# bgmanuel99/Super-Resolution-Images-for-3D-Printing-Defect-Detection

Hardware: AMD Instinct MI355X
Metric: 4x-SR MPix/s on 512x512 LR batch (higher is better)
Workload: dtype bf16

## Files before the change

super-resolution-images-for-3d-printing-defect-detection_amd/csrc/attention.hip:

```cpp
#include "common.h"

#include <cstdlib>

namespace {

constexpr int KV_TILE = 64;

template <typename T> struct AT;
template <> struct AT<float>  { static constexpr int PITCH = KV_TILE * 4 + 4; };

struct AttnParams {
    const char* qkv; int64_t cs; int qoff, koff, voff;
    char* o; int64_t o_cs; int o_coff;
    int N;
    const float* knorm;
};

__device__ __forceinline__ float xhalf(float v) { return __shfl_xor(v, 32); }

__global__ void __launch_bounds__(256, 2) attn_f32_kernel(AttnParams p) {
    constexpr int PITCH = AT<float>::PITCH;
    __shared__ __attribute__((aligned(16))) char vt[32 * PITCH];

    const int tid = threadIdx.x, lane = tid & 63, wave = tid >> 6, r = lane & 31, h = lane >> 5;
    const int b = blockIdx.y;
    const int N = p.N;
    const float* base = reinterpret_cast<const float*>(p.qkv) + (int64_t)b * N * p.cs;
    const int q = blockIdx.x * 128 + wave * 32 + r;
    const int qc = q < N ? q : N - 1;

    float qf[4];
    {
        const float* qp = base + (int64_t)qc * p.cs + p.qoff;
#pragma unroll
        for (int j = 0; j < 4; ++j) qf[j] = qp[2 * j + h];
    }

    f32x16 oacc;
#pragma unroll
    for (int e = 0; e < 16; ++e) oacc[e] = 0.f;
    float m_run = -INFINITY, l_run = 0.f;

    const int skey = tid >> 2, soct = tid & 3;

    for (int k0 = 0; k0 < N; k0 += KV_TILE) {
        __syncthreads();
        {
            const int key = k0 + skey;
            const float* vp = base + (int64_t)(key < N ? key : N - 1) * p.cs + p.voff + soct * 8;
            f32x4 v0 = *reinterpret_cast<const f32x4*>(vp), v1 = *reinterpret_cast<const f32x4*>(vp + 4);
#pragma unroll
            for (int e = 0; e < 4; ++e) {
                *reinterpret_cast<float*>(vt + (soct * 8 + e) * PITCH + skey * 4) = v0[e];
                *reinterpret_cast<float*>(vt + (soct * 8 + 4 + e) * PITCH + skey * 4) = v1[e];
            }
        }
        __syncthreads();
#pragma unroll
        for (int sub = 0; sub < KV_TILE / 32; ++sub) {
            const int kb = k0 + sub * 32;
            if (kb >= N) break;
            f32x16 s;
#pragma unroll
            for (int e = 0; e < 16; ++e) s[e] = 0.f;
            {
                const int key = kb + r;
                const float* kp = base + (int64_t)(key < N ? key : N - 1) * p.cs + p.koff;
#pragma unroll
                for (int j = 0; j < 4; ++j) s = __builtin_amdgcn_mfma_f32_32x32x2f32(kp[2 * j + h], qf[j], s, 0, 0, 0);
            }
            float mx = -INFINITY;
#pragma unroll
            for (int i = 0; i < 16; ++i) {
                const int key = kb + (i & 3) + 8 * (i >> 2) + 4 * h;
                if (key >= N) s[i] = -INFINITY;
                mx = fmaxf(mx, s[i]);
            }
            mx = fmaxf(mx, xhalf(mx));
            const float m_new = fmaxf(m_run, mx);
            const float alpha = __expf(m_run - m_new);
            float psum = 0.f;
#pragma unroll
            for (int i = 0; i < 16; ++i) { s[i] = __expf(s[i] - m_new); psum += s[i]; }
            l_run = l_run * alpha + psum;
            m_run = m_new;
#pragma unroll
            for (int e = 0; e < 16; ++e) oacc[e] *= alpha;
#pragma unroll
            for (int i = 0; i < 16; ++i) {
                const int krow = sub * 32 + (i & 3) + 8 * (i >> 2);
                const float va = *reinterpret_cast<const float*>(vt + r * PITCH + (krow + 4 * h) * 4);
                oacc = __builtin_amdgcn_mfma_f32_32x32x2f32(va, s[i], oacc, 0, 0, 0);
            }
        }
    }
    const float l_tot = l_run + xhalf(l_run);
    const float inv = 1.f / l_tot;
    if (q < N) {
        float* op = reinterpret_cast<float*>(p.o) + ((int64_t)b * N + q) * p.o_cs + p.o_coff;
#pragma unroll
        for (int g = 0; g < 4; ++g) {
            const int d0 = 8 * g + 4 * h;
            f32x4 t = {oacc[4 * g] * inv, oacc[4 * g + 1] * inv, oacc[4 * g + 2] * inv, oacc[4 * g + 3] * inv};
            *reinterpret_cast<f32x4*>(op + d0) = t;
        }
    }
}

constexpr int KT2 = 128;
constexpr int PITCH2 = KT2 * 2 + 8;

__global__ void __launch_bounds__(64) attn_knorm_kernel(const bf16_t* qkv, int64_t cs, int koff, int N, int ngroups, float* out) {
    const int g = blockIdx.x % ngroups, b = blockIdx.x / ngroups, lane = threadIdx.x;
    const bf16_t* base = qkv + (int64_t)b * N * cs + koff;
    float m = 0.f;
#pragma unroll
    for (int t = 0; t < 2; ++t) {
        const int key = g * 128 + t * 64 + lane;
        if (key < N) {
            const bf16x8 k = *reinterpret_cast<const bf16x8*>(base + (int64_t)key * cs);
            float n2 = 0.f;
#pragma unroll
            for (int e = 0; e < 8; ++e) n2 += (float)k[e] * (float)k[e];
            m = fmaxf(m, n2);
        }
    }
#pragma unroll
    for (int o = 32; o > 0; o >>= 1) m = fmaxf(m, __shfl_xor(m, o));
    if (lane == 0) out[(int64_t)b * ngroups + g] = sqrtf(m);
}

template <int QB>
__global__ void __launch_bounds__(256, 3) attn_bf16_kernel(AttnParams p) {
    __shared__ __attribute__((aligned(16))) char vt[32 * PITCH2];
    const int tid = threadIdx.x, lane = tid & 63, wave = tid >> 6, r = lane & 31, h = lane >> 5;
    const int N = p.N;
    constexpr int QW = 64 * QB * 2;
    const int nqt = (N + QW - 1) / QW;
    const int b = blockIdx.x / nqt, qt = blockIdx.x - b * nqt;
    const bf16_t* base = reinterpret_cast<const bf16_t*>(p.qkv) + (int64_t)b * N * p.cs;
    const int cs = (int)p.cs;
    int qi[QB];
    bf16x8 qb[QB];
#pragma unroll
    for (int j = 0; j < QB; ++j) {
        qi[j] = qt * QW + wave * (32 * QB) + j * 32 + r;
        const int qc = qi[j] < N ? qi[j] : N - 1;
        bf16x8 z = {};
        qb[j] = z;
        if (h == 0) qb[j] = *reinterpret_cast<const bf16x8*>(base + (int64_t)qc * cs + p.qoff);
    }
    float qn2 = 0.f;
#pragma unroll
    for (int j = 0; j < QB; ++j) {
        float n2 = 0.f;
#pragma unroll
        for (int e = 0; e < 8; ++e) n2 += (float)qb[j][e] * (float)qb[j][e];
        qn2 = fmaxf(qn2, n2);
    }
#pragma unroll
    for (int o = 32; o > 0; o >>= 1) qn2 = fmaxf(qn2, __shfl_xor(qn2, o));
    const float qmaxv = sqrtf(qn2) * 1.0009765625f;
    const int* knorm_bits = reinterpret_cast<const int*>(p.knorm) + (int64_t)b * ((N + KT2 - 1) / KT2);
    f32x16 oacc[QB];
    bf16x8 sel = {};
    {
        const int m = lane & 15, kg = lane >> 4;
        const bf16_t one = (bf16_t)1.f;
        if ((m == 0 && (kg & 1) == 0) || (m == 1 && (kg & 1) == 1)) sel = bf16x8{one, one, one, one, one, one, one, one};
    }
    f32x4 lacc[QB];
    float m_run[QB];
#pragma unroll
    for (int j = 0; j < QB; ++j) {
        m_run[j] = 0.f; lacc[j] = f32x4{0.f, 0.f, 0.f, 0.f};
#pragma unroll
        for (int e = 0; e < 16; ++e) oacc[j][e] = 0.f;
    }

    const int kp = tid >> 2, oct = tid & 3;
    bf16x8 kneg = {};
    kneg[0] = (bf16_t)-1.f; kneg[1] = (bf16_t)-1.f; kneg[2] = (bf16_t)-1.f;
    auto load_k = [&](int kb) {
        int l;
        asm volatile("v_mbcnt_lo_u32_b32 %0, -1, 0\n\tv_mbcnt_hi_u32_b32 %0, -1, %0" : "=v"(l));
        bf16x8 kf = kneg;
        const int key = kb + (l & 31);
        if (l < 32) kf = *reinterpret_cast<const bf16x8*>(base + (int64_t)(key < N ? key : N - 1) * cs + p.koff);
        return kf;
    };
    bf16x8 knext = load_k(0);
    f32x16 zero16;
#pragma unroll
    for (int e = 0; e < 16; ++e) zero16[e] = 0.f;
    struct { } false_c; struct { int x; } true_c{0};
    auto hmax = [](float v) {
        const unsigned u = __builtin_bit_cast(unsigned, v);
        const auto sw = __builtin_amdgcn_permlane32_swap(u, u, false, false);
        return fmaxf(__builtin_bit_cast(float, (unsigned)sw[0]), __builtin_bit_cast(float, (unsigned)sw[1]));
    };
    auto tile = [&](const bf16x8 kf, const int sub, const int kb, auto ragged_tag, const bool first) {
        constexpr bool RAGGED = sizeof(ragged_tag) > 1;
        f32x16 s[QB];
        float mx[QB];
#pragma unroll
        for (int j = 0; j < QB; ++j) {
            s[j] = __builtin_amdgcn_mfma_f32_32x32x16_bf16(kf, qb[j], zero16, 0, 0, 0);
            if constexpr (RAGGED) {
#pragma unroll
                for (int i = 0; i < 16; ++i)
                    if (kb + (i & 3) + 8 * (i >> 2) + 4 * h >= N) s[j][i] = -INFINITY;
            }
            float m = fmaxf(fmaxf(s[j][0], s[j][1]), s[j][2]);
#pragma unroll
            for (int i = 3; i + 1 < 16; i += 2) m = fmaxf(fmaxf(m, s[j][i]), s[j][i + 1]);
            m = fmaxf(m, s[j][15]);
            mx[j] = hmax(m);
        }
        bool grew = first;
#pragma unroll
        for (int j = 0; j < QB; ++j) grew = grew || mx[j] > 0.f;
        if (__any(grew)) {
#pragma unroll
            for (int j = 0; j < QB; ++j) {
                const float delta = first ? mx[j] : fmaxf(mx[j], 0.f);
                const float alpha = first ? 1.f : __builtin_amdgcn_exp2f(-delta);
                lacc[j][0] *= alpha;
                lacc[j][1] *= __shfl(alpha, (lane + 16) & 63);
#pragma unroll
                for (int e = 0; e < 16; ++e) oacc[j][e] *= alpha;
#pragma unroll
                for (int i = 0; i < 16; ++i) s[j][i] -= delta;
                m_run[j] += delta;
                if (h == 1) {
                    const bf16_t m1 = (bf16_t)m_run[j];
                    const float r1 = m_run[j] - (float)m1;
                    const bf16_t m2 = (bf16_t)r1;
                    qb[j][0] = m1; qb[j][1] = m2; qb[j][2] = (bf16_t)(r1 - (float)m2);
                }
            }
        }
#pragma unroll
        for (int j = 0; j < QB; ++j) {
#pragma unroll
            for (int i = 0; i < 16; ++i) s[j][i] = __builtin_amdgcn_exp2f(s[j][i]);
        }
#pragma unroll
        for (int ks = 0; ks < 2; ++ks) {
            const char* vrow = vt + r * PITCH2 + (sub * 32 + 16 * ks + 4 * h) * 2;
            const bf16x4 va = *reinterpret_cast<const bf16x4*>(vrow);
            const bf16x4 vb = *reinterpret_cast<const bf16x4*>(vrow + 16);
            const bf16x8 vf = {va[0], va[1], va[2], va[3], vb[0], vb[1], vb[2], vb[3]};
#pragma unroll
            for (int j = 0; j < QB; ++j) {
                bf16x8 pf;
#pragma unroll
                for (int e = 0; e < 8; ++e) pf[e] = (bf16_t)s[j][8 * ks + e];
                oacc[j] = __builtin_amdgcn_mfma_f32_32x32x16_bf16(vf, pf, oacc[j], 0, 0, 0);
                lacc[j] = __builtin_amdgcn_mfma_f32_16x16x32_bf16(sel, pf, lacc[j], 0, 0, 0);
            }
        }
    };

    constexpr float GROW_OK = 40.f;
    auto tile_fast = [&](const bf16x8 kf, const int sub, const bool guard) -> bool {
        f32x16 s[QB];
#pragma unroll
        for (int j = 0; j < QB; ++j) s[j] = __builtin_amdgcn_mfma_f32_32x32x16_bf16(kf, qb[j], zero16, 0, 0, 0);
        if (guard) {
            bool risky = false;
#pragma unroll
            for (int j = 0; j < QB; ++j) {
                float m = fmaxf(fmaxf(s[j][0], s[j][1]), s[j][2]);
#pragma unroll
                for (int i = 3; i + 1 < 16; i += 2) m = fmaxf(fmaxf(m, s[j][i]), s[j][i + 1]);
                m = fmaxf(m, s[j][15]);
                risky = risky || m > GROW_OK;
            }
            if (__any(risky)) return false;
        }
#pragma unroll
        for (int j = 0; j < QB; ++j) {
#pragma unroll
            for (int i = 0; i < 16; ++i) s[j][i] = __builtin_amdgcn_exp2f(s[j][i]);
        }
#pragma unroll
        for (int ks = 0; ks < 2; ++ks) {
            const char* vrow = vt + r * PITCH2 + (sub * 32 + 16 * ks + 4 * h) * 2;
            const bf16x4 va = *reinterpret_cast<const bf16x4*>(vrow);
            const bf16x4 vb = *reinterpret_cast<const bf16x4*>(vrow + 16);
            const bf16x8 vf = {va[0], va[1], va[2], va[3], vb[0], vb[1], vb[2], vb[3]};
#pragma unroll
            for (int j = 0; j < QB; ++j) {
                bf16x8 pf;
#pragma unroll
                for (int e = 0; e < 8; ++e) pf[e] = (bf16_t)s[j][8 * ks + e];
                oacc[j] = __builtin_amdgcn_mfma_f32_32x32x16_bf16(vf, pf, oacc[j], 0, 0, 0);
                lacc[j] = __builtin_amdgcn_mfma_f32_16x16x32_bf16(sel, pf, lacc[j], 0, 0, 0);
            }
        }
        return true;
    };
    auto thresh_of_wave = [&]() -> int {
        float m = m_run[0];
#pragma unroll
        for (int j = 1; j < QB; ++j) m = fminf(m, m_run[j]);
#pragma unroll
        for (int o = 32; o > 0; o >>= 1) m = fminf(m, __shfl_xor(m, o));
        const float lim = GROW_OK + m;
        const float th = !(lim >= 0.f) ? -1.f : (qmaxv > 0.f ? lim / qmaxv * 0.9990234375f : INFINITY);
        return __builtin_amdgcn_readfirstlane(__builtin_bit_cast(int, th));
    };
    int thresh_bits = __builtin_amdgcn_readfirstlane(__builtin_bit_cast(int, -1.f));
    auto stage_v = [&](const int k0) {
        __syncthreads();
#pragma unroll
        for (int part = 0; part < KT2 / 128; ++part) {
            const int ka = k0 + part * 128 + 2 * kp, kbb = ka + 1;
            if (ka - 2 * kp >= N) break;
            const bf16x8 va = *reinterpret_cast<const bf16x8*>(base + (int64_t)(ka < N ? ka : N - 1) * cs + p.voff + oct * 8);
            const bf16x8 vb = *reinterpret_cast<const bf16x8*>(base + (int64_t)(kbb < N ? kbb : N - 1) * cs + p.voff + oct * 8);
#pragma unroll
            for (int e = 0; e < 8; ++e) {
                typedef bf16_t bf16x2 __attribute__((ext_vector_type(2)));
                bf16x2 pr = {va[e], vb[e]};
                *reinterpret_cast<bf16x2*>(vt + (oct * 8 + e) * PITCH2 + (part * 64 + kp) * 4) = pr;
            }
        }
        __syncthreads();
    };
    auto slow_tiles = [&](const int k0, const int sub0, bf16x8 kf) {
        for (int sub = sub0; sub < KT2 / 32; ++sub) {
            const int kb = k0 + sub * 32;
            if (kb >= N) break;
            if (sub != sub0) { kf = knext; knext = load_k(kb + 32); }
            if (kb + 32 <= N) tile(kf, sub, kb, false_c, kb == 0);
            else tile(kf, sub, kb, true_c, kb == 0);
        }
    };

    for (int k0 = 0; k0 < N; k0 += KT2) {
        stage_v(k0);
        int sub = 0;
        bf16x8 kf = knext;
        const bool full = k0 != 0 && k0 + KT2 <= N;
        if (full) {
            const bool guard = !(knorm_bits[k0 / KT2] <= thresh_bits);
#pragma unroll
            for (; sub < KT2 / 32; ++sub) {
                kf = knext;
                knext = load_k(k0 + sub * 32 + 32);
                if (!tile_fast(kf, sub, guard)) break;
            }
        } else {
            knext = load_k(k0 + 32);
        }
        if (sub < KT2 / 32) {
            slow_tiles(k0, sub, kf);
            thresh_bits = thresh_of_wave();
        }
    }
#pragma unroll
    for (int j = 0; j < QB; ++j) {
        const float l0 = __shfl(lacc[j][0], r & 15), l1 = __shfl(lacc[j][1], r & 15);
        const float inv = 1.f / ((r >> 4) ? l1 : l0);
        if (qi[j] < N) {
            bf16_t* op = reinterpret_cast<bf16_t*>(p.o) + ((int64_t)b * N + qi[j]) * p.o_cs + p.o_coff;
#pragma unroll
            for (int g = 0; g < 4; ++g) {
                bf16x4 t = {(bf16_t)(oacc[j][4 * g] * inv), (bf16_t)(oacc[j][4 * g + 1] * inv), (bf16_t)(oacc[j][4 * g + 2] * inv),
                            (bf16_t)(oacc[j][4 * g + 3] * inv)};
                *reinterpret_cast<bf16x4*>(op + 8 * g + 4 * h) = t;
            }
        }
    }
}

}

int attention_launch(sr_ctx* ctx, int dtype, const void* qkv, int64_t cs, int qoff, int koff, int voff, int B, int N,
                     void* o, int64_t o_cs, int o_coff, hipStream_t st) {
    if (B <= 0 || N <= 0) return ctx->fail(SR_ERR_INVALID, "attention: empty tensor");
    const int esz = dtype_size(dtype);
    if ((cs * esz) % 16 || (qoff * esz) % 16 || (koff * esz) % 16 || (voff * esz) % 16 || (o_cs * esz) % 16 || (o_coff * esz) % 16)
        return ctx->fail(SR_ERR_INVALID, "attention: views must be 16-byte aligned");
    AttnParams p{static_cast<const char*>(qkv), cs, qoff, koff, voff, static_cast<char*>(o), o_cs, o_coff, N, nullptr};
    dim3 grid((unsigned)((N + 127) / 128), (unsigned)B);
    if (dtype != SR_DTYPE_BF16 && dtype != SR_DTYPE_F32) return ctx->fail(SR_ERR_INVALID, "attention: dtype must be f32 or bf16");
    const int rec = ctx->prof_open(dtype == SR_DTYPE_BF16 ? "attn<bf16>" : "attn<f32>", 2.0 * B * (double)N * N * 40.0,
                                   (double)B * N * 80.0 * esz, st);
    if (dtype == SR_DTYPE_BF16) {
        static const int qb_env = [] { const char* e = getenv("SR355_ATTN_QB"); return e ? atoi(e) : 2; }();
        const int QBr = qb_env == 1 ? 1 : 2;
        const int64_t nwg = (int64_t)B * ((N + 128 * QBr - 1) / (128 * QBr));
        const int ngroups = (N + KT2 - 1) / KT2;
        if (nwg >= (1ll << 31) || (int64_t)B * ngroups >= (1ll << 31)) { ctx->prof_close(rec, st); return ctx->fail(SR_ERR_INVALID, "attention: too many workgroups for one launch"); }
        float* kn = static_cast<float*>(ctx->arena(ctx->attn_kn, sizeof(float) * (size_t)B * ngroups, st));
        if (!kn) { ctx->prof_close(rec, st); return SR_ERR_OOM; }
        p.knorm = kn;
        hipLaunchKernelGGL(attn_knorm_kernel, dim3((unsigned)((int64_t)B * ngroups)), dim3(64), 0, st, reinterpret_cast<const bf16_t*>(qkv) + 0, cs, koff, N, ngroups, kn);
        if (QBr == 1) hipLaunchKernelGGL(attn_bf16_kernel<1>, dim3((unsigned)nwg), dim3(256), 0, st, p);
        else hipLaunchKernelGGL(attn_bf16_kernel<2>, dim3((unsigned)nwg), dim3(256), 0, st, p);
    }
    else hipLaunchKernelGGL(attn_f32_kernel, grid, dim3(256), 0, st, p);
    ctx->prof_close(rec, st);
    SR_HIP(ctx, hipGetLastError());
    return SR_OK;
}
```

Baseline: 112.0.

## Add software-pipelined fast path for guarded key groups via LDS-staged K

Adds a PIPE variant of the bf16 attention kernel that stages a whole group of K rows into shared memory alongside V, then runs a software-pipelined loop where the next QK^T MFMA is issued before the current P·V MFMAs. It is used for full key groups whose norm bound shows no running-max rescaling is needed. That lets it skip the per-tile max tracking and the break check. The goal is to hide MFMA and global-load latency in the common fast case. In exchange it adds LDS usage and a reload of the register K prefetch after pipelined groups, and the launcher now reads its env vars on every call. The new path is on by default, with SR355_ATTN_LEGACY selecting the old path.

```diff
diff --git a/super-resolution-images-for-3d-printing-defect-detection_amd/csrc/attention.hip b/super-resolution-images-for-3d-printing-defect-detection_amd/csrc/attention.hip
--- a/super-resolution-images-for-3d-printing-defect-detection_amd/csrc/attention.hip
+++ b/super-resolution-images-for-3d-printing-defect-detection_amd/csrc/attention.hip
@@ -1,6 +1,7 @@
 #include "common.h"
 
 #include <cstdlib>
+#include <cstring>
 
 namespace {
 
@@ -130,9 +131,10 @@
     if (lane == 0) out[(int64_t)b * ngroups + g] = sqrtf(m);
 }
 
-template <int QB>
+template <int QB, bool PIPE>
 __global__ void __launch_bounds__(256, 3) attn_bf16_kernel(AttnParams p) {
     __shared__ __attribute__((aligned(16))) char vt[32 * PITCH2];
+    __shared__ __attribute__((aligned(16))) char kimg[PIPE ? (KT2 / 32) * 64 * 16 : 16];
     const int tid = threadIdx.x, lane = tid & 63, wave = tid >> 6, r = lane & 31, h = lane >> 5;
     const int N = p.N;
     constexpr int QW = 64 * QB * 2;
@@ -190,6 +192,9 @@
         return kf;
     };
     bf16x8 knext = load_k(0);
+    if constexpr (PIPE) {
+        if (tid < KT2) *reinterpret_cast<bf16x8*>(kimg + ((tid >> 5) * 64 + 32 + (tid & 31)) * 16) = kneg;
+    }
     f32x16 zero16;
 #pragma unroll
     for (int e = 0; e < 16; ++e) zero16[e] = 0.f;
@@ -301,6 +306,41 @@
         }
         return true;
     };
+    auto group_pipe = [&]() {
+        int l;
+        asm volatile("v_mbcnt_lo_u32_b32 %0, -1, 0\n\tv_mbcnt_hi_u32_b32 %0, -1, %0" : "=v"(l));
+        const char* kl = kimg + l * 16;
+        bf16x8 kf = *reinterpret_cast<const bf16x8*>(kl);
+        f32x16 sa = __builtin_amdgcn_mfma_f32_32x32x16_bf16(kf, qb[0], zero16, 0, 0, 0), sb;
+        bf16x8 vf[2];
+#pragma unroll
+        for (int u = 0; u < 4 * QB; ++u) {
+            const int t = u / QB, j = u % QB;
+            if (u + 1 < 4 * QB) {
+                const int tn = (u + 1) / QB, jn = (u + 1) % QB;
+                if (jn == 0) kf = *reinterpret_cast<const bf16x8*>(kl + tn * 64 * 16);
+                sb = __builtin_amdgcn_mfma_f32_32x32x16_bf16(kf, qb[jn], zero16, 0, 0, 0);
+            }
+            if (j == 0) {
+#pragma unroll
+                for (int ks = 0; ks < 2; ++ks) {
+                    const char* vrow = vt + r * PITCH2 + (t * 32 + 16 * ks + 4 * h) * 2;
+                    const bf16x4 va = *reinterpret_cast<const bf16x4*>(vrow);
+                    const bf16x4 vb = *reinterpret_cast<const bf16x4*>(vrow + 16);
+                    vf[ks] = bf16x8{va[0], va[1], va[2], va[3], vb[0], vb[1], vb[2], vb[3]};
+                }
+            }
+#pragma unroll
+            for (int ks = 0; ks < 2; ++ks) {
+                bf16x8 pf;
+#pragma unroll
+                for (int e = 0; e < 8; ++e) pf[e] = (bf16_t)__builtin_amdgcn_exp2f(sa[8 * ks + e]);
+                oacc[j] = __builtin_amdgcn_mfma_f32_32x32x16_bf16(vf[ks], pf, oacc[j], 0, 0, 0);
+                lacc[j] = __builtin_amdgcn_mfma_f32_16x16x32_bf16(sel, pf, lacc[j], 0, 0, 0);
+            }
+            sa = sb;
+        }
+    };
     auto thresh_of_wave = [&]() -> int {
         float m = m_run[0];
 #pragma unroll
@@ -312,8 +352,16 @@
         return __builtin_amdgcn_readfirstlane(__builtin_bit_cast(int, th));
     };
     int thresh_bits = __builtin_amdgcn_readfirstlane(__builtin_bit_cast(int, -1.f));
+    bool knext_stale = false;
     auto stage_v = [&](const int k0) {
         __syncthreads();
+        if constexpr (PIPE) {
+            if (tid < KT2) {
+                const int key = k0 + tid;
+                *reinterpret_cast<bf16x8*>(kimg + ((tid >> 5) * 64 + (tid & 31)) * 16) =
+                    *reinterpret_cast<const bf16x8*>(base + (int64_t)(key < N ? key : N - 1) * cs + p.koff);
+            }
+        }
 #pragma unroll
         for (int part = 0; part < KT2 / 128; ++part) {
             const int ka = k0 + part * 128 + 2 * kp, kbb = ka + 1;
@@ -340,6 +388,15 @@
     };
 
     for (int k0 = 0; k0 < N; k0 += KT2) {
+        if constexpr (PIPE) {
+            if (k0 != 0 && k0 + KT2 <= N && knorm_bits[k0 / KT2] <= thresh_bits) {
+                stage_v(k0);
+                group_pipe();
+                knext_stale = true;
+                continue;
+            }
+            if (knext_stale) { knext = load_k(k0); knext_stale = false; }
+        }
         stage_v(k0);
         int sub = 0;
         bf16x8 kf = knext;
@@ -390,8 +447,10 @@
     const int rec = ctx->prof_open(dtype == SR_DTYPE_BF16 ? "attn<bf16>" : "attn<f32>", 2.0 * B * (double)N * N * 40.0,
                                    (double)B * N * 80.0 * esz, st);
     if (dtype == SR_DTYPE_BF16) {
-        static const int qb_env = [] { const char* e = getenv("SR355_ATTN_QB"); return e ? atoi(e) : 2; }();
-        const int QBr = qb_env == 1 ? 1 : 2;
+        const char* qb_env = getenv("SR355_ATTN_QB");
+        const char* legacy_env = getenv("SR355_ATTN_LEGACY");
+        const int QBr = qb_env && atoi(qb_env) == 1 ? 1 : 2;
+        const bool legacy = legacy_env && *legacy_env && strcmp(legacy_env, "0") != 0;
         const int64_t nwg = (int64_t)B * ((N + 128 * QBr - 1) / (128 * QBr));
         const int ngroups = (N + KT2 - 1) / KT2;
         if (nwg >= (1ll << 31) || (int64_t)B * ngroups >= (1ll << 31)) { ctx->prof_close(rec, st); return ctx->fail(SR_ERR_INVALID, "attention: too many workgroups for one launch"); }
@@ -399,8 +458,10 @@
         if (!kn) { ctx->prof_close(rec, st); return SR_ERR_OOM; }
         p.knorm = kn;
         hipLaunchKernelGGL(attn_knorm_kernel, dim3((unsigned)((int64_t)B * ngroups)), dim3(64), 0, st, reinterpret_cast<const bf16_t*>(qkv) + 0, cs, koff, N, ngroups, kn);
-        if (QBr == 1) hipLaunchKernelGGL(attn_bf16_kernel<1>, dim3((unsigned)nwg), dim3(256), 0, st, p);
-        else hipLaunchKernelGGL(attn_bf16_kernel<2>, dim3((unsigned)nwg), dim3(256), 0, st, p);
+        if (QBr == 1 && legacy) hipLaunchKernelGGL((attn_bf16_kernel<1, false>), dim3((unsigned)nwg), dim3(256), 0, st, p);
+        else if (QBr == 1) hipLaunchKernelGGL((attn_bf16_kernel<1, true>), dim3((unsigned)nwg), dim3(256), 0, st, p);
+        else if (legacy) hipLaunchKernelGGL((attn_bf16_kernel<2, false>), dim3((unsigned)nwg), dim3(256), 0, st, p);
+        else hipLaunchKernelGGL((attn_bf16_kernel<2, true>), dim3((unsigned)nwg), dim3(256), 0, st, p);
     }
     else hipLaunchKernelGGL(attn_f32_kernel, grid, dim3(256), 0, st, p);
     ctx->prof_close(rec, st);
```

New measurement: 113.8 (median of 6 runs). 1.7% higher.
